# Image-Processing-Systems-Laboratory/DeepInPainting

Measured on AMD Instinct MI355X. Metric: train images/sec at 256x256, batch 8/GPU, 1/2/4/8 MI355X; IPSR layer ms, higher is better.
Workload: dtype f32; 1 GPU; BASELINE config 2: 256x256 synthetic images, 128x128 centre mask (M=256 of N=1024 feature positions), batch 8/GPU, fp32, full IPSR training step; global_batch=8, parallelism=dp1, dropout=True, conv_math=fp32, vgg16=seeded random init (no pretrained weights offline)

## Files before the change

deepinpainting_amd/csrc/smallmap.hip:

```cpp
#include <algorithm>

#include "ipsr_common.h"

namespace ipsr {

typedef float f32x16 __attribute__((ext_vector_type(16)));
typedef float f32x4v __attribute__((ext_vector_type(4)));

__global__ void __launch_bounds__(256) sm_to_cn_kernel(const float* __restrict__ x, int B, int C, int HW, int Tp, float* __restrict__ out)
{
    const int n = blockIdx.x * 256 + threadIdx.x, c = blockIdx.y;
    if (n >= Tp) return;
    float v = 0.0f;
    if (n < B * HW) { const int b = n / HW, p = n - b * HW; v = x[((size_t)b * C + c) * HW + p]; }
    out[(size_t)c * Tp + n] = v;
}

__global__ void __launch_bounds__(256) sm_to_nc_kernel(const float* __restrict__ x, int B, int C, int HW, float* __restrict__ out)
{
    const int c = blockIdx.x * 256 + threadIdx.x, n = blockIdx.y;
    if (c >= C) return;
    float v = 0.0f;
    if (n < B * HW) { const int b = n / HW, p = n - b * HW; v = x[((size_t)b * C + c) * HW + p]; }
    out[(size_t)n * C + c] = v;
// ... 354 lines not shown
    };
    auto mma = [&](const Set& s) {
#pragma unroll
        for (int u = 0; u < G; ++u)
#pragma unroll
            for (int j = 0; j < 4; ++j) acc[j] = __builtin_amdgcn_mfma_f32_32x32x2f32(s.av[u], s.b[u][j], acc[j], 0, 0, 0);
    };
    sm_stream<Set>(cdiv_dev(Pp, 2 * G), load, mma);
#pragma unroll
    for (int e = 0; e < 16; ++e) {
        const int row = (e & 3) + 8 * (e >> 2) + 4 * h;
        *reinterpret_cast<f32x4v*>(dW + (size_t)(r0 + row) * Q + q0 + 4 * m) = f32x4v{acc[0][e], acc[1][e], acc[2][e], acc[3][e]};
    }
}

constexpr int SM_WRW_GATHER_MAX_POS = 32;
static bool sm_staged(int op, int P)
{
    const int forced = debug_option(3);
    return forced == 1 || (forced != 2 && op == 1 && P > SM_WRW_GATHER_MAX_POS);
}

struct SmPlan { int P, Tp, Pp, Q, nb, ngroups, nslab, per_slab; size_t a_floats, b_floats, m_floats, total_bytes; };

static int sm_plan(int op, int B, int R, int Cq, int Ho, int Wo, int Hf, int Wf, int k, int st, int pad, int dil, SmPlan* p)
{
    if (op < 0 || op > 2) return fail(IPSR_ERR_INVALID, "small-map convolution: op %d", op);
    if (k < 1 || k > 4 || st < 1 || st > 2 || dil < 1 || pad < 0) return fail(IPSR_ERR_UNSUPPORTED, "small-map convolution: k%d s%d p%d d%d", k, st, pad, dil);
    if (Ho != (Hf + 2 * pad - dil * (k - 1) - 1) / st + 1 || Wo != (Wf + 2 * pad - dil * (k - 1) - 1) / st + 1)
        return fail(IPSR_ERR_INVALID, "small-map convolution: %dx%d is not the output grid of %dx%d under k%d s%d p%d d%d", Ho, Wo, Hf, Wf, k, st, pad, dil);
    p->P = B * Ho * Wo;
    p->Q = Cq * k * k;
    if (p->Q % 128 != 0) return fail(IPSR_ERR_UNSUPPORTED, "small-map convolution: %d x %d taps is not a multiple of 128", Cq, k * k);
    if (R % 32 != 0) return fail(IPSR_ERR_UNSUPPORTED, "small-map convolution: %d weight rows are not a multiple of 32", R);
    if (p->P > 1024) return fail(IPSR_ERR_UNSUPPORTED, "small-map convolution: %d positions (made for <= 1024)", p->P);
    const int blocks = (p->P + 31) / 32;
    p->nb = blocks >= 4 ? 4 : (blocks == 3 ? 4 : blocks);
    if (op == 0 && p->nb == 4) p->nb = 2;
    p->ngroups = (blocks + p->nb - 1) / p->nb;
    p->Tp = p->ngroups * p->nb * 32;
    p->Pp = (p->P + 1) & ~1;
    p->a_floats = p->b_floats = p->m_floats = 0;
    p->nslab = 1; p->per_slab = 0;
    const size_t w_bytes = (size_t)R * p->Q * 4;
    if (op == 0) {
        const int qb = p->Q / 128;
        const size_t slab_bytes = (size_t)p->Q * p->Tp * 4;
        const int cap = (int)std::max<size_t>(1, w_bytes / slab_bytes);
        int ns = std::max(1, std::min({R / 64, cap, (256 + qb * p->ngroups - 1) / (qb * p->ngroups)}));
        p->per_slab = (((R + 4 * ns - 1) / (4 * ns)) + 1) & ~1;
        p->nslab = (R + 4 * p->per_slab - 1) / (4 * p->per_slab);
        p->b_floats = (size_t)R * p->Tp;
        p->m_floats = (size_t)p->nslab * p->Q * p->Tp;
    } else if (op == 2) {
        const int rb = R / 32;
        const size_t slab_bytes = (size_t)R * p->Tp * 4;
        const int cap = (int)std::max<size_t>(1, w_bytes / slab_bytes);
        int ns = std::max(1, std::min({p->Q / 256, cap, (256 + rb * p->ngroups - 1) / (rb * p->ngroups)}));
// ... 16 lines not shown
    return p.total_bytes;
}

int launch_smallmap(int op, const float* a, const float* b2, float* out, int B, int R, int Cq, int Ho, int Wo, int Hf, int Wf,
                    int k, int st_, int pad, int dil, void* ws, size_t ws_bytes, hipStream_t st)
{
    SmPlan p;
    if (int rc = sm_plan(op, B, R, Cq, Ho, Wo, Hf, Wf, k, st_, pad, dil, &p)) return rc;
    if (ws_bytes < p.total_bytes) return fail(IPSR_ERR_WORKSPACE, "small-map convolution: workspace %zu < %zu", ws_bytes, p.total_bytes);
    Carver cv(ws, ws_bytes);
    float* A = cv.take<float>(p.a_floats);
    float* Bv = cv.take<float>(p.b_floats);
    float* Mo = cv.take<float>(p.m_floats);
    const size_t largest = 4 * std::max({(size_t)R * p.Q, (size_t)B * Cq * Hf * Wf, (size_t)R * p.Tp, (size_t)p.Q * p.Tp, (size_t)p.Pp * p.Q});
    if (largest >= SM_OFF) return fail(IPSR_ERR_UNSUPPORTED, "small-map convolution: an operand of %zu bytes (made for < 2 GiB)", largest);
    const bool staged = sm_staged(op, p.P);
    const SmGeo g = {p.P, R, Cq, Ho, Wo, Hf, Wf, k, st_, pad, dil};
    if (op == 0) {
        if (staged) sm_to_cn_kernel<<<dim3(cdiv(p.Tp, 256), R), 256, 0, st>>>(a, B, R, Ho * Wo, p.Tp, Bv);
        const float* in = staged ? Bv : a;
        const int HW = staged ? 0 : Ho * Wo;
        const dim3 grid(p.Q / 128, p.nslab, p.ngroups);
        if (p.nb == 1) sm_data_kernel<1><<<grid, 256, 0, st>>>(b2, in, R, p.Q, p.Tp, p.per_slab, p.P, HW, Mo);
        else sm_data_kernel<2><<<grid, 256, 0, st>>>(b2, in, R, p.Q, p.Tp, p.per_slab, p.P, HW, Mo);
        if (int rc = check_launch("sm_data_kernel")) return rc;
        const size_t total = (size_t)B * Cq * Hf * Wf;
        const unsigned cgrid = (unsigned)((total + 255) / 256);
        const size_t slab_bytes = (size_t)p.Q * p.Tp * 4, m_bytes = slab_bytes * p.nslab;
        const bool wide = !debug_option(4) && m_bytes < SM_OFF && (k == 3 || k == 4) && p.nslab <= 8;
        if (wide && k == 3) sm_col2im_wide_kernel<3, 8><<<cgrid, 256, 0, st>>>(Mo, p.nslab, (unsigned)slab_bytes, (unsigned)m_bytes, B, Cq, Hf, Wf, Ho, Wo, st_, pad, dil, p.Tp, out);
        else if (wide && p.nslab <= 4) sm_col2im_wide_kernel<4, 4><<<cgrid, 256, 0, st>>>(Mo, p.nslab, (unsigned)slab_bytes, (unsigned)m_bytes, B, Cq, Hf, Wf, Ho, Wo, st_, pad, dil, p.Tp, out);
        else if (wide) sm_col2im_wide_kernel<4, 8><<<cgrid, 256, 0, st>>>(Mo, p.nslab, (unsigned)slab_bytes, (unsigned)m_bytes, B, Cq, Hf, Wf, Ho, Wo, st_, pad, dil, p.Tp, out);
        else sm_col2im_kernel<<<cgrid, 256, 0, st>>>(Mo, p.nslab, (size_t)p.Q * p.Tp, B, Cq, Hf, Wf, Ho, Wo, k, st_, pad, dil, p.Tp, out);
        return check_launch("sm_col2im_kernel");
    }
    const int K = staged ? 0 : k;
    if (op == 2) {
        if (staged) sm_im2col_cn_kernel<<<dim3(cdiv(p.Tp, 256), p.Q), 256, 0, st>>>(a, B, Cq, Hf, Wf, Ho, Wo, k, st_, pad, dil, p.Tp, Bv);
        const float* x = staged ? Bv : a;
        const dim3 grid(R / 32, p.nslab, p.ngroups);
#define SM_FWD_K(NB)                                                                                                                                   \
    switch (K) {                                                                                                                                       \
    case 0: sm_fwd_kernel<NB, 0><<<grid, 256, 0, st>>>(b2, x, R, p.Q, p.Tp, p.per_slab, g, Mo); break;                                                 \
    case 1: sm_fwd_kernel<NB, 1><<<grid, 256, 0, st>>>(b2, x, R, p.Q, p.Tp, p.per_slab, g, Mo); break;                                                 \
    case 2: sm_fwd_kernel<NB, 2><<<grid, 256, 0, st>>>(b2, x, R, p.Q, p.Tp, p.per_slab, g, Mo); break;                                                 \
    case 3: sm_fwd_kernel<NB, 3><<<grid, 256, 0, st>>>(b2, x, R, p.Q, p.Tp, p.per_slab, g, Mo); break;                                                 \
    default: sm_fwd_kernel<NB, 4><<<grid, 256, 0, st>>>(b2, x, R, p.Q, p.Tp, p.per_slab, g, Mo); break;                                                \
    }
        if (p.nb == 1) { SM_FWD_K(1) }
        else if (p.nb == 2) { SM_FWD_K(2) }
        else { SM_FWD_K(4) }
// ... 47 lines not shown
```

deepinpainting_amd/models/IPSR.py:

```python
import os
from collections import OrderedDict

import torch

from . import networks
from .base_model import BaseModel
from .vgg16 import Vgg16
from .. import dist as ipsr_dist


class IPSR(BaseModel):
    def name(self):
        return 'IPSRModel'

    def initialize(self, opt):
        BaseModel.initialize(self, opt)
        self.opt = opt
        self.isTrain = opt.isTrain
        self.strict_reference = bool(getattr(opt, 'strict_reference', False))
        self.batch_vgg = bool(getattr(opt, 'batch_vgg', False))
        self.batch_disc = bool(getattr(opt, 'batch_disc', True))
        self.amp_bf16 = bool(getattr(opt, 'amp_bf16', False))
        from . import hipconv
        hipconv.set_conv_math(fp32=getattr(opt, 'conv_math', 'fp32'), bf16=getattr(opt, 'conv_math_bf16', 'bf16x3'))
# ... 27 lines not shown
        self.use_gpu = len(opt.gpu_ids) > 0

        self.netG, self.Cosis_list, self.Cosis_list2, self.CSA_model = networks.define_G(
            opt.input_nc_g, opt.output_nc, opt.ngf, opt.which_model_netG, opt, self.mask_global, opt.norm,
            opt.use_dropout, opt.init_type, self.gpu_ids, opt.init_gain)
        self.netP, _, _, _ = networks.define_G(
            opt.input_nc, opt.output_nc, opt.ngf, opt.which_model_netP, opt, self.mask_global, opt.norm,
            opt.use_dropout, opt.init_type, self.gpu_ids, opt.init_gain)
        self.CSA_model[0].corr_bf16 = self.amp_bf16 and bool(getattr(opt, 'bf16_corr', True)) and self.device.type == 'cuda'
        if self.isTrain:
            use_sigmoid = opt.gan_type == 'vanilla'
            self.netD = networks.define_D(opt.input_nc, opt.ndf, opt.which_model_netD, opt.n_layers_D, opt.norm,
                                          use_sigmoid, opt.init_type, self.gpu_ids, opt.init_gain)
            self.netF = networks.define_D(opt.input_nc, opt.ndf, opt.which_model_netF, opt.n_layers_D, opt.norm,
                                          use_sigmoid, opt.init_type, self.gpu_ids, opt.init_gain)

        if not self.isTrain or opt.continue_train:
            print('Loading pre-trained network!')
            self.load_network(self.netG, 'G', opt.which_epoch)
            self.load_network(self.netP, 'P', opt.which_epoch)
            if self.isTrain:
                self.load_network(self.netD, 'D', opt.which_epoch)
                self.load_network(self.netF, 'F', opt.which_epoch)

        self.criterionGAN = networks.GANLoss(gan_type=opt.gan_type)
        self.criterionL1 = torch.nn.L1Loss()
        self._gt_latent = None
        self._reducer_D = self._reducer_G = None

        if self.isTrain:
# ... 236 lines not shown
```

deepinpainting_amd/models/hipconv.py:

```python
import os
from collections import namedtuple

import torch
import torch.nn as nn
import torch.nn.functional as F

from .. import _lib, ops
from .. import dist as ipsr_dist

_FORCE = None
_MATH = {"fp32": "fp32", "bf16": "bf16x3"}


def set_conv_math(fp32=None, bf16=None):
    from .. import ops as _ops
    for key, val in (("fp32", fp32), ("bf16", bf16)):
        if val is not None:
            if val not in _ops.MATH_CODE or (key == "bf16" and val in _ops.DIRECT_PASSES):
                raise ValueError("conv math must be one of %s" % sorted(k for k in _ops.MATH_CODE if k))
            _MATH[key] = val
    _SEL.clear()


_DIRECT_DILATED = False
# ... 44 lines not shown
    v = _ENV.get(name)
    if v is None:
        v = _ENV[name] = os.environ.get(name, default)
    return v


def reload_env():
    _ENV.clear()
    _SEL.clear()


def _mode():
    return _FORCE or _env("IPSR_CONV_ENGINE", "auto")


def select(op, B, Cin, H, W, Cout, k, stride, pad, dil, bf16=False):
    key = (0, _FORCE, op, B, Cin, H, W, Cout, k, stride, pad, dil, bf16)
    eng = _SEL.get(key)
    if eng is None:
        eng = _SEL[key] = _select_any(op, (op in (ops.CONVT_FWD, ops.CONVT_BWD_DATA), B, Cin, H, W, Cout, k, stride, pad, dil), bf16)
    return eng


def _select_any(op, lay, bf16):
    eng = _select(op, lay)
    transposed, B, Cin, H, W, Cout, k, stride, pad, dil = lay
    if not bf16:
        eng = _direct_opt_in("data", eng, op, lay)
    elif not (_bf16_wins(eng, Cin, H, W, Cout) or _ENGINES[eng].fp32_copies):
        if _mode() == "auto" and _thin_wins(op, lay, True):
            eng = "thin"
        elif _mode() == "auto" and _env("IPSR_NO_THIN", "0") != "1" and op == ops.CONV_FWD and Cin == 3 and (k, stride, pad, dil) == (4, 2, 1, 1) and H * W >= 4096 \
                and engine_takes("thin_f2m", "data", op, lay, True):
            eng = "thin_f2m"
        else:
            eng = _bf16_direct(op, lay)
# ... 128 lines not shown
    return g[3] >= 1 and g[4] >= 1 and g[0] * g[3] * g[4] <= int(_env("IPSR_SMALLMAP_MAX_POS", "32")) and engine_takes("smallmap", "data", op, lay, False)


def _smallmap_wrw_wins(lay):
    transposed, B, Cin, H, W, Cout, k, stride, pad, dil = lay
    if k != 4 or stride != 2 or _env("IPSR_NO_SMALLMAP", "0") == "1":
        return False
    g = _smallmap_geometry(lay)
    return g[3] >= 1 and g[4] >= 1 and g[0] * g[3] * g[4] <= 256 and min(Cin, Cout) >= 256 and engine_takes("smallmap", "wrw", None, lay, False)


def _is_k4s1(k, stride, pad, dil):
    return k == 4 and stride == 1 and pad == 1 and dil == 1


def select_wrw(transposed, B, Cin, H, W, Cout, k, stride, pad, dil, bf16=False):
    key = (1, _FORCE, transposed, B, Cin, H, W, Cout, k, stride, pad, dil, bf16)
    eng = _SEL.get(key)
    if eng is None:
        eng = _SEL[key] = _select_wrw_any((transposed, B, Cin, H, W, Cout, k, stride, pad, dil), bf16)
    return eng


def _select_wrw_any(lay, bf16):
    transposed, B, Cin, H, W, Cout, k, stride, pad, dil = lay
    eng = _select_wrw(lay)
    thin = _mode() == "auto" and _env("IPSR_NO_THIN", "0") != "1" and pad == 1 and dil == 1 and (k, stride) in ((3, 1), (4, 2)) and H * W >= 4096 \
        and engine_takes("thin_mfma", "wrw", None, lay, bf16)
    if not bf16:
        eng = "thin_mfma" if thin and eng == "miopen" else _direct_opt_in("wrw", eng, None, lay)
    elif not (_bf16_wins(eng, Cin, H, W, Cout, True) or _ENGINES[eng].fp32_copies):
        eng = "thin_mfma" if thin else _bf16_direct_wrw(lay)
    return eng if engine_takes(eng, "wrw", None, lay, bf16) else "miopen"


def _bf16_direct_wrw(lay):
# ... 201 lines not shown
        _wino_dil_takes, bf16_io=True, sink=True, wrw_x_as_dy=True),
    "wino_s2": _Engine(
        lambda op, inp, w, lay, math, out_dtype, param: ops.conv4x4s2_winograd(_s2_mode(op), inp, w, lay[1], *_s2_geometry(lay), math=math, out_dtype=out_dtype),
        lambda x, dy, lay, math, sink: ops.conv4x4s2_winograd(ops.S2_WEIGHT_GRAD, *_fine_coarse(x, dy, lay), out=sink, math=math),
        _wino_s2_takes, bf16_io=True, sink=True, wrw_x_as_dy=True),
    "thin": _Engine(
        lambda op, inp, w, lay, math, out_dtype, param: ops.conv3x3_thin(op, inp, w, lay[1:5], lay[5], out_dtype=out_dtype),
        takes=lambda kind, op, lay, bf16: kind == "data" and lay[6:] == _K3 and ops.thin_supported(op, *lay[2:6])),
    "thin_f2m": _Engine(
        lambda op, inp, w, lay, math, out_dtype, param: ops.conv_thin_f2m_mfma(op, inp, w, lay[1:5], lay[5], lay[6], lay[7], out_dtype=out_dtype),
        takes=lambda kind, op, lay, bf16: kind == "data" and lay[8:] == (1, 1) and ops.thin_f2m_mfma_supported(op, *lay[1:8])),
    "thin_mfma": _Engine(
        None, _thin_mfma_wrw, sink=True,
        takes=lambda kind, op, lay, bf16: kind == "wrw" and lay[8:] == (1, 1) and ops.thin_wrw_mfma_supported(*lay[:8])),
    "smallmap": _Engine(
        lambda op, inp, w, lay, math, out_dtype, param: ops.conv_smallmap(_smallmap_op(op), inp, w, *_smallmap_geometry(lay)),
        lambda x, dy, lay, math, sink: ops.conv_smallmap(ops.SM_WRW, *((x, dy) if lay[0] else (dy, x)), *_smallmap_geometry(lay), out=sink),
        lambda kind, op, lay, bf16: ops.smallmap_supported(_smallmap_op(op) if kind == "data" else ops.SM_WRW, *_smallmap_geometry(lay)),
        fp32_copies=True, sink=True),
    "direct": _Engine(
        lambda op, inp, w, lay, math, out_dtype, param: ops.conv2d(op, inp, w, lay[1:5], *lay[5:]),
        takes=lambda kind, op, lay, bf16: kind == "data" and ops.conv2d_supported(op, *lay[1:])),
    "one": _Engine(
        lambda op, inp, w, lay, math, out_dtype, param: ops.conv_to_one(inp, w, lay[8]),
        lambda x, dy, lay, math, sink: ops.conv_to_one_wrw(x, dy, lay[6], lay[8], out=sink),
        lambda kind, op, lay, bf16: not lay[0] and lay[5] == 1 and (kind == "wrw" or op == ops.CONV_FWD) and ops.conv_to_one_supported(*lay[1:5], *lay[6:]),
        fp32_copies=True, sink=True),
    "bf16d": _Engine(_bf16d_data, _bf16d_wrw, _bf16d_takes, bf16_io=True, sink=True, wrw_x_as_dy=True),
    "bf16x3d": _Engine(_bf16x3d_data, takes=_bf16x3d_takes),
    "bf16x3w": _Engine(None, _bf16x3w_wrw, _bf16x3w_takes, sink=True),
    "miopen": _Engine(),
}


def _run_data(eng, op, inp, w, lay, math, out_dtype, param=None):
    e = _ENGINES[eng]
    if e.fp32_copies:
        return e.data(op, inp.float(), w, lay, math, torch.float32, param).to(out_dtype)
    return e.data(op, inp, w, lay, math, out_dtype, param)


def _run_wrw(eng, x, dy, w, lay, math):
    e = _ENGINES[eng]
    sink = ipsr_dist.grad_sink_for(w.data_ptr(), w.shape) if e.sink else None
    if e.fp32_copies:
        x, dy = x.float(), dy.float()
    elif e.wrw_x_as_dy and x.dtype != dy.dtype:
        x = x.to(dy.dtype)
    return e.wrw(x, dy, lay, math, sink)


def _miopen_forward(x, w, transposed, stride, pad, dil):
    if x.dtype != w.dtype and not torch.is_autocast_enabled():
        w = w.to(x.dtype)
    return F.conv_transpose2d(x, w, None, stride, pad, 0, 1, dil) if transposed else F.conv2d(x, w, None, stride, pad, dil)


def _miopen_backward(dy, x, w, transposed, stride, pad, dil, which):
    dt = dy.dtype
    out = torch.ops.aten.convolution_backward(dy, x if x.dtype == dt else x.to(dt), w if w.dtype == dt else w.to(dt), None, [stride, stride],
                                              [pad, pad], [dil, dil], transposed, [0, 0], 1, which)
    return out[0], (out[1].to(w.dtype) if out[1] is not None else None)


class _HipConv(torch.autograd.Function):

    @staticmethod
    def forward(ctx, x, w, lay, eng_fwd, math, act):
        transposed, B, Cin, H, W, Cout, k, stride, pad, dil = lay
        xc = x.contiguous()
        if eng_fwd == "miopen":
            y = _miopen_forward(xc, w, transposed, stride, pad, dil)
        else:
            y = _run_data(eng_fwd, ops.CONVT_FWD if transposed else ops.CONV_FWD, xc, w, lay, math, act)
        ctx.save_for_backward(xc, w)
        ctx.lay, ctx.geom = lay, (transposed, k, stride, pad, dil, Cout)
        ctx.math, ctx.bf16 = math, act == torch.bfloat16
        if _check_hook is not None:
            _check_hook("forward", eng_fwd, ctx.geom, (xc, w), y)
        return y

    @staticmethod
    def backward(ctx, dy):
        x, w = ctx.saved_tensors
        lay, math, bf16 = ctx.lay, ctx.math, ctx.bf16
        transposed, B, Cin, H, W, Cout, k, stride, pad, dil = lay
        dy = dy.contiguous()
        if bf16 and dy.dtype != torch.bfloat16:
            dy = dy.to(torch.bfloat16)
        dx = dw = None
        if ctx.needs_input_grad[0]:
            op = ops.CONVT_BWD_DATA if transposed else ops.CONV_BWD_DATA
            eng = select(op, B, Cin, H, W, Cout, k, stride, pad, dil, bf16)
            if eng == "miopen":
                dx = _miopen_backward(dy, x, w, transposed, stride, pad, dil, [True, False, False])[0]
                if dx.dtype != x.dtype:
                    dx = dx.to(x.dtype)
            else:
                dx = _run_data(eng, op, dy, w, lay, math, x.dtype)
            if _check_hook is not None:
                _check_hook("input_grad", eng, ctx.geom, (dy, x, w), dx)
        if ctx.needs_input_grad[1]:
            weng = select_wrw(transposed, B, Cin, H, W, Cout, k, stride, pad, dil, bf16)
            if weng == "miopen":
                dw = _miopen_backward(dy, x, w, transposed, stride, pad, dil, [False, True, False])[1]
            else:
                dw = _run_wrw(weng, x, dy, w, lay, math)
            if _check_hook is not None:
                _check_hook("weight_grad", weng, ctx.geom, (dy, x, w), dw)
        return dx, dw, None, None, None, None


def _geometry(m):
    ks, st, pd, dl = m.kernel_size, m.stride, m.padding, m.dilation
    if m.groups != 1 or ks[0] != ks[1] or st[0] != st[1] or pd[0] != pd[1] or dl[0] != dl[1] or isinstance(pd, str):
        return None
    if isinstance(m, nn.ConvTranspose2d) and tuple(m.output_padding) != (0, 0):
        return None
    if getattr(m, "padding_mode", "zeros") != "zeros":
        return None
    return ks[0], st[0], pd[0], dl[0]


def _layer_of(m, x, w):
    g = _geometry(m)
    if g is None or not x.is_cuda or x.dim() != 4 or w.dtype != torch.float32 or x.dtype not in (torch.float32, torch.bfloat16):
        return None
    amp = _amp_bf16()
    if not amp and torch.is_autocast_enabled():
        return None
    transposed = isinstance(m, nn.ConvTranspose2d)
    B, Cin, H, W = x.shape
    return (transposed, B, Cin, H, W, w.shape[1] if transposed else w.shape[0]) + g, amp or x.dtype == torch.bfloat16


def conv_math(bf16):
    return _MATH["bf16" if bf16 else "fp32"]


def _engines_of(lay, bf16, dx=True, dw=True):
    transposed, B, Cin, H, W, Cout, k, stride, pad, dil = lay
    fop, bop = (ops.CONVT_FWD, ops.CONVT_BWD_DATA) if transposed else (ops.CONV_FWD, ops.CONV_BWD_DATA)
    return (select(fop, B, Cin, H, W, Cout, k, stride, pad, dil, bf16),
            select(bop, B, Cin, H, W, Cout, k, stride, pad, dil, bf16) if dx else "miopen",
            select_wrw(transposed, B, Cin, H, W, Cout, k, stride, pad, dil, bf16) if dw else "miopen")


def any_engine(m, x):
    lb = _layer_of(m, x, m.weight)
    if lb is None:
        return False
    return _engines_of(*lb) != ("miopen",) * 3


def conv_nobias(m, x, weight=None):
    w = m.weight if weight is None else weight
    lb = _layer_of(m, x, w)
    if lb is not None:
        lay, bf16 = lb
        act = torch.bfloat16 if bf16 else torch.float32
        math = _MATH["bf16" if bf16 else "fp32"]
        grad = torch.is_grad_enabled()
        engs = _engines_of(lay, bf16, grad and x.requires_grad, grad and w.requires_grad)
        if grad and (x.requires_grad or w.requires_grad):
            if engs != ("miopen",) * 3:
                return _HipConv.apply(x, w, lay, engs[0], math, act)
        elif engs[0] != "miopen":
            return _run_data(engs[0], ops.CONVT_FWD if lay[0] else ops.CONV_FWD, x.contiguous(), w.detach(), lay, math, act, param=w)
    if isinstance(m, nn.ConvTranspose2d):
        return F.conv_transpose2d(x, w, None, m.stride, m.padding, m.output_padding, m.groups, m.dilation)
    return F.conv2d(x, w, None, m.stride, m.padding, m.dilation, m.groups)
```

deepinpainting_amd/ops.py:

```python
import contextlib
import threading
import weakref
from collections import namedtuple

import torch

from . import _lib

_ws_cache = {}


def _stream():
    return torch._C._cuda_getCurrentRawStream(torch._C._cuda_getDevice())


def _workspace(nbytes, device):
    key = (device.index, _stream())
    buf = _ws_cache.get(key)
    if buf is None or buf.numel() < nbytes:
        buf = torch.empty(max(int(nbytes), 1 << 20), dtype=torch.uint8, device=device)
        _ws_cache[key] = buf
    return buf


# ... 858 lines not shown
    Cs = small.shape[1]
    if tuple(small.shape) != (B, Cs, Hb * stride, Wb * stride):
        raise RuntimeError("conv_thin_wrw_mfma: narrow tensor %s does not match wide %s at stride %d" % (tuple(small.shape), tuple(big.shape), stride))
    L = _lib.lib()
    g = _result(out, (Kb, Cs, k, k), torch.float32, x.device, "conv_thin_wrw_mfma")
    ws = _probed_workspace(L, L.ipsr_conv_thin_wrw_mfma_workspace_bytes(B, Kb, Cs, Hb, Wb, k, stride), x.device,
                           "ipsr_conv_thin_wrw_mfma: Kb=%d Cs=%d %dx%d k%d s%d", (Kb, Cs, Hb, Wb, k, stride))
    _lib.check(L.ipsr_conv_thin_wrw_mfma(big.data_ptr(), small.data_ptr(), g.data_ptr(), B, Kb, Cs, Hb, Wb, k, stride, int(big.dtype == torch.bfloat16) | (2 if small.dtype == torch.bfloat16 else 0),
                                         ws.data_ptr(), ws.numel(), _stream()), "ipsr_conv_thin_wrw_mfma")
    return g


SM_DATA, SM_WRW, SM_FWD = 0, 1, 2


def smallmap_supported(op, B, R, Cq, Ho, Wo, Hf, Wf, k, stride, pad, dil):
    return _lib.lib().ipsr_conv_smallmap_workspace_bytes(op, B, R, Cq, Ho, Wo, Hf, Wf, k, stride, pad, dil) > 0


def conv_smallmap(op, a, b, B, R, Cq, Ho, Wo, Hf, Wf, k, stride, pad, dil, out=None):
    a = _req(a, torch.float32, "operand a")
    b = _req(b, torch.float32, "operand b")
    coarse, fine, wsh = (B, R, Ho, Wo), (B, Cq, Hf, Wf), (R, Cq, k, k)
    want = {SM_DATA: (coarse, wsh, fine), SM_WRW: (coarse, fine, wsh), SM_FWD: (fine, wsh, coarse)}[op]
    if tuple(a.shape) != want[0] or tuple(b.shape) != want[1]:
        raise RuntimeError("conv_smallmap op %d: operands %s / %s do not match %s / %s" % (op, tuple(a.shape), tuple(b.shape), want[0], want[1]))
    out = _result(out, want[2], torch.float32, a.device, "conv_smallmap")
    L = _lib.lib()
    ws = _probed_workspace(L, L.ipsr_conv_smallmap_workspace_bytes(op, B, R, Cq, Ho, Wo, Hf, Wf, k, stride, pad, dil), a.device,
                           "ipsr_conv_smallmap: op %d R=%d Cq=%d %dx%d -> %dx%d k%d s%d p%d d%d", (op, R, Cq, Hf, Wf, Ho, Wo, k, stride, pad, dil))
    _lib.check(L.ipsr_conv_smallmap(op, a.data_ptr(), b.data_ptr(), out.data_ptr(), B, R, Cq, Ho, Wo, Hf, Wf, k, stride, pad, dil,
                                    ws.data_ptr(), ws.numel(), _stream()), "ipsr_conv_smallmap")
    return out


def conv3x3_winograd_wrw(transposed, x, dy, Cout, out=None, math=None):
    x, x_bf = _act(x, "conv input")
    dy, dy_bf = _act(dy, "grad_output")
    if x_bf != dy_bf:
        raise TypeError("conv3x3_winograd_wrw: x and dy must have the same dtype")
    B, Cin, H, W = x.shape
    if tuple(dy.shape) != (B, Cout, H, W):
        raise RuntimeError("conv3x3_winograd_wrw: grad_output %s does not match %s" % (tuple(dy.shape), (B, Cout, H, W)))
# ... 104 lines not shown
```

deepinpainting_amd/options.py:

```python


class Option(object):
    def __init__(self, **overrides):
        self.batchSize = 1
        self.fineSize = 256
        self.input_nc = 3
        self.input_nc_g = 6
        self.output_nc = 3
        self.ngf = 64
        self.ndf = 64
        self.which_model_netD = 'basic'
        self.which_model_netF = 'feature'
        self.which_model_netG = 'unet_ipsr'
        self.which_model_netP = 'unet_256'
        self.triple_weight = 1
        self.name = 'IPSR_inpainting'
        self.n_layers_D = '3'
        self.gpu_ids = [0]
        self.model = 'ipsr_net'
        self.checkpoints_dir = './checkpoints'
        self.norm = 'instance'
        self.fixed_mask = 1
        self.use_dropout = True
        self.init_type = 'normal'
# ... 17 lines not shown
        self.display_freq = 1000
        self.print_freq = 50
        self.save_latest_freq = 5000
        self.save_epoch_freq = 1
        self.continue_train = False
        self.epoch_count = 1
        self.phase = 'train'
        self.which_epoch = ''
        self.niter = 20
        self.niter_decay = 100
        self.beta1 = 0.5
        self.lr = 0.0002
        self.lr_policy = 'lambda'
        self.lr_decay_iters = 50
        self.isTrain = True
        for k, v in overrides.items():
            setattr(self, k, v)
```

include/ipsr_hip.h:

```cpp
#ifndef IPSR_HIP_H
#define IPSR_HIP_H

#include <stddef.h>
#include <stdint.h>

#ifdef __cplusplus
extern "C" {
#endif

#define IPSR_OK                 0
#define IPSR_ERR_INVALID       -1
#define IPSR_ERR_UNSUPPORTED   -2
#define IPSR_ERR_WORKSPACE     -3
#define IPSR_ERR_LAUNCH        -4

int ipsr_abi_version(void);
const char* ipsr_last_error(void);

size_t ipsr_feat_mask_workspace_bytes(int H, int W, int layers);
int ipsr_feat_mask(const uint8_t* mask, int H, int W, int layers, float threshold,
                   uint8_t* feat, void* ws, size_t ws_bytes, void* stream);

int ipsr_index_prep(const uint8_t* feat, int h, int w, int patch, int stride, int mask_thred,
                    int32_t* flag , int32_t* mask_point_idx , int32_t* count ,
// ... 81 lines not shown
int ipsr_conv3x3_winograd_wrw(int transposed, const float* x, const float* dy, float* dw, int B, int Cin, int H, int W, int Cout,
                              void* ws, size_t ws_bytes, void* stream);

size_t ipsr_conv4x4_dilated_winograd_workspace_bytes(int mode, int B, int Cin, int H, int W, int Cout);
int ipsr_conv4x4_dilated_winograd(int mode, const float* a, const float* b, float* out, int B, int Cin, int H, int W, int Cout,
                                  void* ws, size_t ws_bytes, void* stream);

size_t ipsr_conv4x4_winograd_workspace_bytes(int geom, int mode, int B, int Cin, int H, int W, int Cout);
int ipsr_conv4x4_winograd(int geom, int mode, const float* a, const float* b, float* out, int B, int Cin, int H, int W, int Cout,
                          void* ws, size_t ws_bytes, void* stream);

size_t ipsr_conv4x4s2_winograd_workspace_bytes(int mode, int B, int Kc, int Cf, int nh, int nw);
int ipsr_conv4x4s2_winograd(int mode, const float* a, const float* b, float* out, int B, int Kc, int Cf, int nh, int nw,
                            void* ws, size_t ws_bytes, void* stream);

size_t ipsr_conv_smallmap_workspace_bytes(int op, int B, int R, int Cq, int Ho, int Wo, int Hf, int Wf, int k, int stride, int pad, int dil);
int ipsr_conv_smallmap(int op, const float* a, const float* b, float* out, int B, int R, int Cq, int Ho, int Wo, int Hf, int Wf,
                       int k, int stride, int pad, int dil, void* ws, size_t ws_bytes, void* stream);

int ipsr_conv3x3_thin(int op, const float* in, const float* w, const float* bias, int relu, float* out, int B, int I, int O, int H, int W,
                      long so, long si, int flip, void* stream);
size_t ipsr_conv3x3_thin_wrw_workspace_bytes(int B, int Cb, int Cs, int H, int W);
int ipsr_conv3x3_thin_io(int op, const void* in, const float* w, const float* bias, int relu, void* out, int B, int I, int O, int H, int W,
                         long so, long si, int flip, int io, void* stream);
int ipsr_conv3x3_thin_wrw_io(const void* big, const void* small, float* g, int B, int Cb, int Cs, int H, int W, int io,
                             void* ws, size_t ws_bytes, void* stream);
int ipsr_conv_thin_f2m_mfma_supported(int B, int Cs, int O, int Ho, int Wo, int k, int stride);
int ipsr_conv_thin_f2m_mfma(const void* in, const float* w, const float* bias, int relu, void* out, int B, int Cs, int O, int Ho, int Wo, int k, int stride,
                            long so, long si, int flip, int io, void* stream);
size_t ipsr_conv_thin_wrw_mfma_workspace_bytes(int B, int Kb, int Cs, int Hb, int Wb, int k, int stride);
// ... 78 lines not shown
```

Before: 353.7 images/sec.

## Add tiled MFMA small-map conv kernel and route MIOpen k4 layers to it

Adds a 128x128x16 LDS-tiled MFMA GEMM kernel for small-map convolution forward and backward-data. It double-buffers the weight tiles, uses direct global-to-LDS DMA in the backward-data path, and split-K partials, with a sum or col2im pass afterwards. The Python selector gains a per-module 'reach' option, on by default up to 1024 positions. With it, k=4 layers with at least 256 channels that previously fell back to MIOpen are sent to the smallmap engine (tiled or streaming) according to a position-count regime table. The aim is to beat MIOpen on mid-sized maps, at the cost of extra split-K partial traffic and a reduction pass.

```diff
diff --git a/deepinpainting_amd/csrc/smallmap.hip b/deepinpainting_amd/csrc/smallmap.hip
--- a/deepinpainting_amd/csrc/smallmap.hip
+++ b/deepinpainting_amd/csrc/smallmap.hip
@@ -392,6 +392,142 @@
     }
 }
 
+typedef const __attribute__((address_space(1))) void* sm_gptr_t;
+typedef __attribute__((address_space(3))) void* sm_lptr_t;
+constexpr int SMT_BM = 128, SMT_BN = 128, SMT_BK = 16, SMT_NBUF = 2, SMT_SLOT = 2 * SMT_BK * SMT_BM;
+
+template <bool FWD, int K>
+__global__ void __launch_bounds__(256, 4) sm_tiled_kernel(const float* __restrict__ Wm, const float* __restrict__ X, int R, int Q, int Tp, int m_tiles,
+                                                          int ksplit, int stages_per_split, int nstage, SmGeo g, float* __restrict__ part)
+{
+    __shared__ __attribute__((aligned(16))) float lds[SMT_NBUF * SMT_SLOT];
+    const int tid = threadIdx.x;
+    const int lane = tid & 63, wave = __builtin_amdgcn_readfirstlane(tid >> 6);
+    const int wm = wave >> 1, wn = wave & 1, r = lane & 31, h = lane >> 5;
+    const int M = FWD ? R : Q;
+
+    const unsigned L = xcd_remap(blockIdx.x, gridDim.x);
+    const int mt = L % m_tiles, ks = (L / m_tiles) % ksplit, nt = L / (m_tiles * ksplit);
+    const int m0 = mt * SMT_BM, n0 = nt * SMT_BN;
+    const int s_lo = ks * stages_per_split;
+    const int ns = min(nstage, s_lo + stages_per_split) - s_lo;
+
+    const int gpar = wave >> 1, gn = n0 + (tid & 127);
+    const int HW = g.Ho * g.Wo;
+    const __amdgpu_buffer_rsrc_t xrs = sm_rsrc(X, (unsigned)(g.P / HW) * (FWD ? g.C * g.Hf * g.Wf : R * HW) * 4u);
+    const SmPos pos(g, gn);
+    const unsigned icol = gn < g.P ? (unsigned)((gn / HW) * R * HW + gn % HW) * 4u : SM_OFF;
+    float breg[8];
+    auto gather = [&](int s) {
+        const unsigned row0 = (unsigned)((s_lo + s) * SMT_BK + 8 * gpar);
+#pragma unroll
+        for (int jj = 0; jj < 8; ++jj)
+            breg[jj] = sm_ld(xrs, FWD ? sm_tap_off<K>(g, pos, row0 + jj, 1u) : icol + (row0 + jj) * (unsigned)HW * 4u);
+    };
+    auto store_b = [&](int s) {
+        float* bt = lds + (s & (SMT_NBUF - 1)) * SMT_SLOT + SMT_BK * SMT_BM + (tid & 127);
+#pragma unroll
+        for (int jj = 0; jj < 8; ++jj) bt[(jj + 8 * gpar) * SMT_BM] = breg[jj];
+    };
+
+    const int dma_row = lane >> 5, dma_col = (lane & 31) * 4;
+    const float* wbase = Wm + (size_t)s_lo * SMT_BK * Q + m0 + dma_col;
+    auto dma_piece = [&](int s, int q) {
+        const int slot = (s & (SMT_NBUF - 1)) * SMT_SLOT + q * 2 * SMT_BM;
+        const float* src = wbase + ((size_t)s * SMT_BK + 2 * q + dma_row) * Q;
+        __builtin_amdgcn_global_load_lds((sm_gptr_t)src, (sm_lptr_t)&lds[slot], 16, 0, 0);
+    };
+    auto dma_stage = [&](int s) {
+        dma_piece(s, wave);
+        dma_piece(s, wave + 4);
+    };
+    const __amdgpu_buffer_rsrc_t wrs = sm_rsrc(Wm, (unsigned)R * Q * 4u);
+    const int arow = tid >> 2, akc = tid & 3;
+    unsigned aoff[2];
+#pragma unroll
+    for (int i = 0; i < 2; ++i) {
+        const int row = m0 + arow + 64 * i;
+        aoff[i] = sm_off((unsigned)(min(row, R - 1) * Q + s_lo * SMT_BK + 4 * akc) * 4u, row < R);
+    }
+    f32x4v areg[2];
+    auto load_a = [&](int s) {
+#pragma unroll
+        for (int i = 0; i < 2; ++i) areg[i] = sm_ld4(wrs, aoff[i] + (unsigned)(s * SMT_BK) * 4u);
+    };
+    auto store_a = [&](int s) {
+        float* at = lds + (s & (SMT_NBUF - 1)) * SMT_SLOT + 4 * akc * SMT_BM + arow;
+#pragma unroll
+        for (int i = 0; i < 2; ++i)
+#pragma unroll
+            for (int j = 0; j < 4; ++j) at[j * SMT_BM + 64 * i] = areg[i][j];
+    };
+
+    f32x16 acc[2][2];
+#pragma unroll
+    for (int i = 0; i < 2; ++i)
+#pragma unroll
+        for (int j = 0; j < 2; ++j)
+#pragma unroll
+            for (int e = 0; e < 16; ++e) acc[i][j][e] = 0.0f;
+
+    if constexpr (FWD) load_a(0);
+    else dma_stage(0);
+    gather(0);
+    if constexpr (FWD) store_a(0);
+    store_b(0);
+    asm volatile("s_waitcnt vmcnt(0)" ::: "memory");
+    asm volatile("s_waitcnt lgkmcnt(0)" ::: "memory");
+    __builtin_amdgcn_s_barrier();
+
+    for (int s = 0; s < ns; ++s) {
+        const int cur = s & (SMT_NBUF - 1);
+        const bool more = s + 1 < ns;
+        if (more) {
+            if constexpr (FWD) load_a(s + 1);
+            gather(s + 1);
+        }
+        const float* ta = lds + cur * SMT_SLOT + h * SMT_BM + wm * 32 + r;
+        const float* tb = lds + cur * SMT_SLOT + SMT_BK * SMT_BM + h * SMT_BM + wn * 32 + r;
+        float fa0[3], fa1[3], fb0[3], fb1[3];
+        fa0[0] = ta[0]; fa1[0] = ta[64]; fb0[0] = tb[0]; fb1[0] = tb[64];
+#pragma unroll
+        for (int kk = 0; kk < SMT_BK / 2; ++kk) {
+            const int cs = kk % 3, nx = (kk + 1) % 3;
+            if (kk + 1 < SMT_BK / 2) {
+                const int ro = (kk + 1) * 2 * SMT_BM;
+                fa0[nx] = ta[ro]; fa1[nx] = ta[ro + 64]; fb0[nx] = tb[ro]; fb1[nx] = tb[ro + 64];
+            }
+            if (!FWD && more && kk < 2) dma_piece(s + 1, wave + 4 * kk);
+            __builtin_amdgcn_sched_barrier(0);
+            acc[0][0] = __builtin_amdgcn_mfma_f32_32x32x2f32(fa0[cs], fb0[cs], acc[0][0], 0, 0, 0);
+            acc[0][1] = __builtin_amdgcn_mfma_f32_32x32x2f32(fa0[cs], fb1[cs], acc[0][1], 0, 0, 0);
+            acc[1][0] = __builtin_amdgcn_mfma_f32_32x32x2f32(fa1[cs], fb0[cs], acc[1][0], 0, 0, 0);
+            acc[1][1] = __builtin_amdgcn_mfma_f32_32x32x2f32(fa1[cs], fb1[cs], acc[1][1], 0, 0, 0);
+            __builtin_amdgcn_sched_barrier(0);
+        }
+        asm volatile("s_waitcnt vmcnt(0)" ::: "memory");
+        if (more) {
+            if constexpr (FWD) store_a(s + 1);
+            store_b(s + 1);
+        }
+        asm volatile("s_waitcnt lgkmcnt(0)" ::: "memory");
+        __builtin_amdgcn_s_barrier();
+    }
+
+    float* dst = part + (size_t)ks * M * Tp;
+#pragma unroll
+    for (int jn = 0; jn < 2; ++jn) {
+        const int n = n0 + wn * 32 + jn * 64 + r;
+#pragma unroll
+        for (int im = 0; im < 2; ++im) {
+            const int mb = m0 + wm * 32 + im * 64;
+            if (mb >= M) continue;
+#pragma unroll
+            for (int e = 0; e < 16; ++e) dst[(size_t)(mb + (e & 3) + 8 * (e >> 2) + 4 * h) * Tp + n] = acc[im][jn][e];
+        }
+    }
+}
+
 constexpr int SM_WRW_GATHER_MAX_POS = 32;
 static bool sm_staged(int op, int P)
 {
@@ -399,11 +535,19 @@
     return forced == 1 || (forced != 2 && op == 1 && P > SM_WRW_GATHER_MAX_POS);
 }
 
-struct SmPlan { int P, Tp, Pp, Q, nb, ngroups, nslab, per_slab; size_t a_floats, b_floats, m_floats, total_bytes; };
+constexpr int SM_TILED = 16, SM_TILED_MIN_POS = 33;
+static bool sm_tiled(int op, int flags, int k, int P)
+{
+    return (flags & SM_TILED) && !debug_option(5) && (op == 0 || op == 2) && (k == 3 || k == 4) && P >= SM_TILED_MIN_POS;
+}
+
+struct SmPlan { int P, Tp, Pp, Q, nb, ngroups, nslab, per_slab, m_tiles, nstage; bool tiled; size_t a_floats, b_floats, m_floats, total_bytes; };
 
 static int sm_plan(int op, int B, int R, int Cq, int Ho, int Wo, int Hf, int Wf, int k, int st, int pad, int dil, SmPlan* p)
 {
-    if (op < 0 || op > 2) return fail(IPSR_ERR_INVALID, "small-map convolution: op %d", op);
+    const int flags = op & ~3;
+    op &= 3;
+    if ((flags & ~SM_TILED) || op > 2) return fail(IPSR_ERR_INVALID, "small-map convolution: op %d", op | flags);
     if (k < 1 || k > 4 || st < 1 || st > 2 || dil < 1 || pad < 0) return fail(IPSR_ERR_UNSUPPORTED, "small-map convolution: k%d s%d p%d d%d", k, st, pad, dil);
     if (Ho != (Hf + 2 * pad - dil * (k - 1) - 1) / st + 1 || Wo != (Wf + 2 * pad - dil * (k - 1) - 1) / st + 1)
         return fail(IPSR_ERR_INVALID, "small-map convolution: %dx%d is not the output grid of %dx%d under k%d s%d p%d d%d", Ho, Wo, Hf, Wf, k, st, pad, dil);
@@ -420,6 +564,23 @@
     p->Pp = (p->P + 1) & ~1;
     p->a_floats = p->b_floats = p->m_floats = 0;
     p->nslab = 1; p->per_slab = 0;
+    p->m_tiles = p->nstage = 0;
+    p->tiled = sm_tiled(op, flags, k, p->P);
+    if (p->tiled) {
+        const int M = op == 0 ? p->Q : R, red = op == 0 ? R : p->Q;
+        p->ngroups = (p->P + SMT_BN - 1) / SMT_BN;
+        p->Tp = p->ngroups * SMT_BN;
+        p->m_tiles = (M + SMT_BM - 1) / SMT_BM;
+        p->nstage = red / SMT_BK;
+        const int tiles = p->m_tiles * p->ngroups;
+        int ks = std::max(1, std::min({op == 0 ? 4 : 32, p->nstage / 8, (512 + tiles - 1) / tiles}));
+        if (debug_option(6) > 0) ks = std::min(debug_option(6), p->nstage);
+        p->per_slab = (p->nstage + ks - 1) / ks;
+        p->nslab = (p->nstage + p->per_slab - 1) / p->per_slab;
+        p->m_floats = (size_t)p->nslab * M * p->Tp;
+        p->total_bytes = align_up(p->m_floats * 4, 256) + 768;
+        return IPSR_OK;
+    }
     const size_t w_bytes = (size_t)R * p->Q * 4;
     if (op == 0) {
         const int qb = p->Q / 128;
@@ -466,16 +627,23 @@
     float* Mo = cv.take<float>(p.m_floats);
     const size_t largest = 4 * std::max({(size_t)R * p.Q, (size_t)B * Cq * Hf * Wf, (size_t)R * p.Tp, (size_t)p.Q * p.Tp, (size_t)p.Pp * p.Q});
     if (largest >= SM_OFF) return fail(IPSR_ERR_UNSUPPORTED, "small-map convolution: an operand of %zu bytes (made for < 2 GiB)", largest);
+    op &= 3;
     const bool staged = sm_staged(op, p.P);
     const SmGeo g = {p.P, R, Cq, Ho, Wo, Hf, Wf, k, st_, pad, dil};
+    const unsigned tgrid = (unsigned)(p.m_tiles * p.nslab * p.ngroups);
     if (op == 0) {
-        if (staged) sm_to_cn_kernel<<<dim3(cdiv(p.Tp, 256), R), 256, 0, st>>>(a, B, R, Ho * Wo, p.Tp, Bv);
-        const float* in = staged ? Bv : a;
-        const int HW = staged ? 0 : Ho * Wo;
-        const dim3 grid(p.Q / 128, p.nslab, p.ngroups);
-        if (p.nb == 1) sm_data_kernel<1><<<grid, 256, 0, st>>>(b2, in, R, p.Q, p.Tp, p.per_slab, p.P, HW, Mo);
-        else sm_data_kernel<2><<<grid, 256, 0, st>>>(b2, in, R, p.Q, p.Tp, p.per_slab, p.P, HW, Mo);
-        if (int rc = check_launch("sm_data_kernel")) return rc;
+        if (p.tiled) {
+            sm_tiled_kernel<false, 4><<<tgrid, 256, 0, st>>>(b2, a, R, p.Q, p.Tp, p.m_tiles, p.nslab, p.per_slab, p.nstage, g, Mo);
+            if (int rc = check_launch("sm_tiled_kernel")) return rc;
+        } else {
+            if (staged) sm_to_cn_kernel<<<dim3(cdiv(p.Tp, 256), R), 256, 0, st>>>(a, B, R, Ho * Wo, p.Tp, Bv);
+            const float* in = staged ? Bv : a;
+            const int HW = staged ? 0 : Ho * Wo;
+            const dim3 grid(p.Q / 128, p.nslab, p.ngroups);
+            if (p.nb == 1) sm_data_kernel<1><<<grid, 256, 0, st>>>(b2, in, R, p.Q, p.Tp, p.per_slab, p.P, HW, Mo);
+            else sm_data_kernel<2><<<grid, 256, 0, st>>>(b2, in, R, p.Q, p.Tp, p.per_slab, p.P, HW, Mo);
+            if (int rc = check_launch("sm_data_kernel")) return rc;
+        }
         const size_t total = (size_t)B * Cq * Hf * Wf;
         const unsigned cgrid = (unsigned)((total + 255) / 256);
         const size_t slab_bytes = (size_t)p.Q * p.Tp * 4, m_bytes = slab_bytes * p.nslab;
@@ -487,6 +655,14 @@
         return check_launch("sm_col2im_kernel");
     }
     const int K = staged ? 0 : k;
+    if (op == 2 && p.tiled) {
+        if (k == 3) sm_tiled_kernel<true, 3><<<tgrid, 256, 0, st>>>(b2, a, R, p.Q, p.Tp, p.m_tiles, p.nslab, p.per_slab, p.nstage, g, Mo);
+        else sm_tiled_kernel<true, 4><<<tgrid, 256, 0, st>>>(b2, a, R, p.Q, p.Tp, p.m_tiles, p.nslab, p.per_slab, p.nstage, g, Mo);
+        if (int rc = check_launch("sm_tiled_kernel")) return rc;
+        const size_t total = (size_t)B * R * Ho * Wo;
+        sm_sum_to_nchw_kernel<<<(unsigned)((total + 255) / 256), 256, 0, st>>>(Mo, p.nslab, (size_t)R * p.Tp, B, R, Ho * Wo, p.Tp, out);
+        return check_launch("sm_sum_to_nchw_kernel");
+    }
     if (op == 2) {
         if (staged) sm_im2col_cn_kernel<<<dim3(cdiv(p.Tp, 256), p.Q), 256, 0, st>>>(a, B, Cq, Hf, Wf, Ho, Wo, k, st_, pad, dil, p.Tp, Bv);
         const float* x = staged ? Bv : a;
diff --git a/deepinpainting_amd/models/IPSR.py b/deepinpainting_amd/models/IPSR.py
--- a/deepinpainting_amd/models/IPSR.py
+++ b/deepinpainting_amd/models/IPSR.py
@@ -65,6 +65,12 @@
                                           use_sigmoid, opt.init_type, self.gpu_ids, opt.init_gain)
             self.netF = networks.define_D(opt.input_nc, opt.ndf, opt.which_model_netF, opt.n_layers_D, opt.norm,
                                           use_sigmoid, opt.init_type, self.gpu_ids, opt.init_gain)
+
+        reach = 0 if self.amp_bf16 else int(getattr(opt, 'smallmap_reach', 1024))
+        for net in (self.netG, self.netP) + ((self.netD, self.netF) if self.isTrain else ()):
+            for mod in net.modules():
+                if isinstance(mod, (torch.nn.Conv2d, torch.nn.ConvTranspose2d)):
+                    mod.smallmap_reach = reach or None
 
         if not self.isTrain or opt.continue_train:
             print('Loading pre-trained network!')
diff --git a/deepinpainting_amd/models/hipconv.py b/deepinpainting_amd/models/hipconv.py
--- a/deepinpainting_amd/models/hipconv.py
+++ b/deepinpainting_amd/models/hipconv.py
@@ -82,12 +82,60 @@
     return _FORCE or _env("IPSR_CONV_ENGINE", "auto")
 
 
-def select(op, B, Cin, H, W, Cout, k, stride, pad, dil, bf16=False):
+def select(op, B, Cin, H, W, Cout, k, stride, pad, dil, bf16=False, reach=None):
     key = (0, _FORCE, op, B, Cin, H, W, Cout, k, stride, pad, dil, bf16)
     eng = _SEL.get(key)
     if eng is None:
         eng = _SEL[key] = _select_any(op, (op in (ops.CONVT_FWD, ops.CONVT_BWD_DATA), B, Cin, H, W, Cout, k, stride, pad, dil), bf16)
-    return eng
+    return _reached("data", key, eng, op, bf16, reach) if reach else eng
+
+
+
+
+def _reach_regime(kind, op, lay):
+    transposed, B, Cin, H, W, Cout, k, stride, pad, dil = lay
+    g = _smallmap_geometry(lay)
+    pos = g[0] * g[3] * g[4] if g[3] >= 1 and g[4] >= 1 else 0
+    if pos < 1:
+        return None
+    if kind == "wrw":
+        return None
+    if pos <= 32:
+        return None
+    if k != 4:
+        return None
+    if pos <= 128:
+        return "stream"
+    fwd = _smallmap_op(op) == ops.SM_FWD
+    if pos <= 256:
+        return "tiled" if fwd else "stream"
+    if pos <= 512:
+        return None if fwd and g[1] > 512 else "tiled"
+    return "tiled" if fwd else None
+
+
+def _reached(kind, key, eng, op, bf16, reach):
+    if eng != "miopen" or bf16:
+        return eng
+    rkey = key + (int(reach),)
+    hit = _SEL.get(rkey)
+    if hit is None:
+        lay = ((op in (ops.CONVT_FWD, ops.CONVT_BWD_DATA),) if kind == "data" else ()) + key[3 if kind == "data" else 2:-1]
+        transposed, B, Cin, H, W, Cout, k, stride, pad, dil = lay
+        g = _smallmap_geometry(lay)
+        regime = _reach_regime(kind, op, lay)
+        ok = _mode() == "auto" and _env("IPSR_NO_SMALLMAP", "0") != "1" and regime is not None and k in (3, 4) and min(Cin, Cout) >= 256 \
+            and g[0] * g[3] * g[4] <= int(reach) and bool(_ENGINES["smallmap"].takes(kind, op, lay, False, tiled=regime == "tiled"))
+        hit = _SEL[rkey] = "smallmap" if ok else eng
+    return hit
+
+
+def _via_reach(kind, op, lay, bf16, reach):
+    if not reach or _reach_regime(kind, op, lay) != "tiled":
+        return False
+    if kind == "data":
+        return select(op, *lay[1:], bf16) != "smallmap" and select(op, *lay[1:], bf16, reach=reach) == "smallmap"
+    return select_wrw(*lay, bf16) != "smallmap" and select_wrw(*lay, bf16, reach=reach) == "smallmap"
 
 
 def _select_any(op, lay, bf16):
@@ -246,12 +294,12 @@
     return k == 4 and stride == 1 and pad == 1 and dil == 1
 
 
-def select_wrw(transposed, B, Cin, H, W, Cout, k, stride, pad, dil, bf16=False):
+def select_wrw(transposed, B, Cin, H, W, Cout, k, stride, pad, dil, bf16=False, reach=None):
     key = (1, _FORCE, transposed, B, Cin, H, W, Cout, k, stride, pad, dil, bf16)
     eng = _SEL.get(key)
     if eng is None:
         eng = _SEL[key] = _select_wrw_any((transposed, B, Cin, H, W, Cout, k, stride, pad, dil), bf16)
-    return eng
+    return _reached("wrw", key, eng, None, bf16, reach) if reach else eng
 
 
 def _select_wrw_any(lay, bf16):
@@ -483,9 +531,11 @@
         None, _thin_mfma_wrw, sink=True,
         takes=lambda kind, op, lay, bf16: kind == "wrw" and lay[8:] == (1, 1) and ops.thin_wrw_mfma_supported(*lay[:8])),
     "smallmap": _Engine(
-        lambda op, inp, w, lay, math, out_dtype, param: ops.conv_smallmap(_smallmap_op(op), inp, w, *_smallmap_geometry(lay)),
-        lambda x, dy, lay, math, sink: ops.conv_smallmap(ops.SM_WRW, *((x, dy) if lay[0] else (dy, x)), *_smallmap_geometry(lay), out=sink),
-        lambda kind, op, lay, bf16: ops.smallmap_supported(_smallmap_op(op) if kind == "data" else ops.SM_WRW, *_smallmap_geometry(lay)),
+        lambda op, inp, w, lay, math, out_dtype, param, tiled=False: ops.conv_smallmap(_smallmap_op(op), inp, w, *_smallmap_geometry(lay), tiled=tiled),
+        lambda x, dy, lay, math, sink, tiled=False: ops.conv_smallmap(ops.SM_WRW, *((x, dy) if lay[0] else (dy, x)), *_smallmap_geometry(lay), out=sink,
+                                                                       tiled=tiled),
+        lambda kind, op, lay, bf16, tiled=False: ops.smallmap_supported(_smallmap_op(op) if kind == "data" else ops.SM_WRW, *_smallmap_geometry(lay),
+                                                                         tiled=tiled),
         fp32_copies=True, sink=True),
     "direct": _Engine(
         lambda op, inp, w, lay, math, out_dtype, param: ops.conv2d(op, inp, w, lay[1:5], *lay[5:]),
@@ -502,21 +552,22 @@
 }
 
 
-def _run_data(eng, op, inp, w, lay, math, out_dtype, param=None):
+def _run_data(eng, op, inp, w, lay, math, out_dtype, param=None, tiled=False):
     e = _ENGINES[eng]
+    kw = {"tiled": True} if tiled else {}
     if e.fp32_copies:
-        return e.data(op, inp.float(), w, lay, math, torch.float32, param).to(out_dtype)
-    return e.data(op, inp, w, lay, math, out_dtype, param)
-
-
-def _run_wrw(eng, x, dy, w, lay, math):
+        return e.data(op, inp.float(), w, lay, math, torch.float32, param, **kw).to(out_dtype)
+    return e.data(op, inp, w, lay, math, out_dtype, param, **kw)
+
+
+def _run_wrw(eng, x, dy, w, lay, math, tiled=False):
     e = _ENGINES[eng]
     sink = ipsr_dist.grad_sink_for(w.data_ptr(), w.shape) if e.sink else None
     if e.fp32_copies:
         x, dy = x.float(), dy.float()
     elif e.wrw_x_as_dy and x.dtype != dy.dtype:
         x = x.to(dy.dtype)
-    return e.wrw(x, dy, lay, math, sink)
+    return e.wrw(x, dy, lay, math, sink, **({"tiled": True} if tiled else {}))
 
 
 def _miopen_forward(x, w, transposed, stride, pad, dil):
@@ -535,16 +586,17 @@
 class _HipConv(torch.autograd.Function):
 
     @staticmethod
-    def forward(ctx, x, w, lay, eng_fwd, math, act):
+    def forward(ctx, x, w, lay, eng_fwd, math, act, reach=None):
         transposed, B, Cin, H, W, Cout, k, stride, pad, dil = lay
         xc = x.contiguous()
         if eng_fwd == "miopen":
             y = _miopen_forward(xc, w, transposed, stride, pad, dil)
         else:
-            y = _run_data(eng_fwd, ops.CONVT_FWD if transposed else ops.CONV_FWD, xc, w, lay, math, act)
+            fop = ops.CONVT_FWD if transposed else ops.CONV_FWD
+            y = _run_data(eng_fwd, fop, xc, w, lay, math, act, tiled=eng_fwd == "smallmap" and _via_reach("data", fop, lay, act == torch.bfloat16, reach))
         ctx.save_for_backward(xc, w)
         ctx.lay, ctx.geom = lay, (transposed, k, stride, pad, dil, Cout)
-        ctx.math, ctx.bf16 = math, act == torch.bfloat16
+        ctx.math, ctx.bf16, ctx.reach = math, act == torch.bfloat16, reach
         if _check_hook is not None:
             _check_hook("forward", eng_fwd, ctx.geom, (xc, w), y)
         return y
@@ -552,7 +604,7 @@
     @staticmethod
     def backward(ctx, dy):
         x, w = ctx.saved_tensors
-        lay, math, bf16 = ctx.lay, ctx.math, ctx.bf16
+        lay, math, bf16, reach = ctx.lay, ctx.math, ctx.bf16, ctx.reach
         transposed, B, Cin, H, W, Cout, k, stride, pad, dil = lay
         dy = dy.contiguous()
         if bf16 and dy.dtype != torch.bfloat16:
@@ -560,24 +612,24 @@
         dx = dw = None
         if ctx.needs_input_grad[0]:
             op = ops.CONVT_BWD_DATA if transposed else ops.CONV_BWD_DATA
-            eng = select(op, B, Cin, H, W, Cout, k, stride, pad, dil, bf16)
+            eng = select(op, B, Cin, H, W, Cout, k, stride, pad, dil, bf16, reach=reach)
             if eng == "miopen":
                 dx = _miopen_backward(dy, x, w, transposed, stride, pad, dil, [True, False, False])[0]
                 if dx.dtype != x.dtype:
                     dx = dx.to(x.dtype)
             else:
-                dx = _run_data(eng, op, dy, w, lay, math, x.dtype)
+                dx = _run_data(eng, op, dy, w, lay, math, x.dtype, tiled=eng == "smallmap" and _via_reach("data", op, lay, bf16, reach))
             if _check_hook is not None:
                 _check_hook("input_grad", eng, ctx.geom, (dy, x, w), dx)
         if ctx.needs_input_grad[1]:
-            weng = select_wrw(transposed, B, Cin, H, W, Cout, k, stride, pad, dil, bf16)
+            weng = select_wrw(transposed, B, Cin, H, W, Cout, k, stride, pad, dil, bf16, reach=reach)
             if weng == "miopen":
                 dw = _miopen_backward(dy, x, w, transposed, stride, pad, dil, [False, True, False])[1]
             else:
-                dw = _run_wrw(weng, x, dy, w, lay, math)
+                dw = _run_wrw(weng, x, dy, w, lay, math, tiled=weng == "smallmap" and _via_reach("wrw", None, lay, bf16, reach))
             if _check_hook is not None:
                 _check_hook("weight_grad", weng, ctx.geom, (dy, x, w), dw)
-        return dx, dw, None, None, None, None
+        return dx, dw, None, None, None, None, None
 
 
 def _geometry(m):
@@ -607,19 +659,19 @@
     return _MATH["bf16" if bf16 else "fp32"]
 
 
-def _engines_of(lay, bf16, dx=True, dw=True):
+def _engines_of(lay, bf16, dx=True, dw=True, reach=None):
     transposed, B, Cin, H, W, Cout, k, stride, pad, dil = lay
     fop, bop = (ops.CONVT_FWD, ops.CONVT_BWD_DATA) if transposed else (ops.CONV_FWD, ops.CONV_BWD_DATA)
-    return (select(fop, B, Cin, H, W, Cout, k, stride, pad, dil, bf16),
-            select(bop, B, Cin, H, W, Cout, k, stride, pad, dil, bf16) if dx else "miopen",
-            select_wrw(transposed, B, Cin, H, W, Cout, k, stride, pad, dil, bf16) if dw else "miopen")
+    return (select(fop, B, Cin, H, W, Cout, k, stride, pad, dil, bf16, reach=reach),
+            select(bop, B, Cin, H, W, Cout, k, stride, pad, dil, bf16, reach=reach) if dx else "miopen",
+            select_wrw(transposed, B, Cin, H, W, Cout, k, stride, pad, dil, bf16, reach=reach) if dw else "miopen")
 
 
 def any_engine(m, x):
     lb = _layer_of(m, x, m.weight)
     if lb is None:
         return False
-    return _engines_of(*lb) != ("miopen",) * 3
+    return _engines_of(*lb, reach=getattr(m, "smallmap_reach", None)) != ("miopen",) * 3
 
 
 def conv_nobias(m, x, weight=None):
@@ -630,12 +682,15 @@
         act = torch.bfloat16 if bf16 else torch.float32
         math = _MATH["bf16" if bf16 else "fp32"]
         grad = torch.is_grad_enabled()
-        engs = _engines_of(lay, bf16, grad and x.requires_grad, grad and w.requires_grad)
+        reach = getattr(m, "smallmap_reach", None)
+        engs = _engines_of(lay, bf16, grad and x.requires_grad, grad and w.requires_grad, reach)
         if grad and (x.requires_grad or w.requires_grad):
             if engs != ("miopen",) * 3:
-                return _HipConv.apply(x, w, lay, engs[0], math, act)
+                return _HipConv.apply(x, w, lay, engs[0], math, act, reach)
         elif engs[0] != "miopen":
-            return _run_data(engs[0], ops.CONVT_FWD if lay[0] else ops.CONV_FWD, x.contiguous(), w.detach(), lay, math, act, param=w)
+            fop = ops.CONVT_FWD if lay[0] else ops.CONV_FWD
+            return _run_data(engs[0], fop, x.contiguous(), w.detach(), lay, math, act, param=w,
+                             tiled=engs[0] == "smallmap" and _via_reach("data", fop, lay, bf16, reach))
     if isinstance(m, nn.ConvTranspose2d):
         return F.conv_transpose2d(x, w, None, m.stride, m.padding, m.output_padding, m.groups, m.dilation)
     return F.conv2d(x, w, None, m.stride, m.padding, m.dilation, m.groups)
diff --git a/deepinpainting_amd/ops.py b/deepinpainting_amd/ops.py
--- a/deepinpainting_amd/ops.py
+++ b/deepinpainting_amd/ops.py
@@ -896,11 +896,14 @@
 SM_DATA, SM_WRW, SM_FWD = 0, 1, 2
 
 
-def smallmap_supported(op, B, R, Cq, Ho, Wo, Hf, Wf, k, stride, pad, dil):
-    return _lib.lib().ipsr_conv_smallmap_workspace_bytes(op, B, R, Cq, Ho, Wo, Hf, Wf, k, stride, pad, dil) > 0
-
-
-def conv_smallmap(op, a, b, B, R, Cq, Ho, Wo, Hf, Wf, k, stride, pad, dil, out=None):
+SM_TILED = 16
+
+
+def smallmap_supported(op, B, R, Cq, Ho, Wo, Hf, Wf, k, stride, pad, dil, tiled=False):
+    return _lib.lib().ipsr_conv_smallmap_workspace_bytes(op | (SM_TILED if tiled else 0), B, R, Cq, Ho, Wo, Hf, Wf, k, stride, pad, dil) > 0
+
+
+def conv_smallmap(op, a, b, B, R, Cq, Ho, Wo, Hf, Wf, k, stride, pad, dil, out=None, tiled=False):
     a = _req(a, torch.float32, "operand a")
     b = _req(b, torch.float32, "operand b")
     coarse, fine, wsh = (B, R, Ho, Wo), (B, Cq, Hf, Wf), (R, Cq, k, k)
@@ -909,6 +912,7 @@
         raise RuntimeError("conv_smallmap op %d: operands %s / %s do not match %s / %s" % (op, tuple(a.shape), tuple(b.shape), want[0], want[1]))
     out = _result(out, want[2], torch.float32, a.device, "conv_smallmap")
     L = _lib.lib()
+    op |= SM_TILED if tiled else 0
     ws = _probed_workspace(L, L.ipsr_conv_smallmap_workspace_bytes(op, B, R, Cq, Ho, Wo, Hf, Wf, k, stride, pad, dil), a.device,
                            "ipsr_conv_smallmap: op %d R=%d Cq=%d %dx%d -> %dx%d k%d s%d p%d d%d", (op, R, Cq, Hf, Wf, Ho, Wo, k, stride, pad, dil))
     _lib.check(L.ipsr_conv_smallmap(op, a.data_ptr(), b.data_ptr(), out.data_ptr(), B, R, Cq, Ho, Wo, Hf, Wf, k, stride, pad, dil,
diff --git a/deepinpainting_amd/options.py b/deepinpainting_amd/options.py
--- a/deepinpainting_amd/options.py
+++ b/deepinpainting_amd/options.py
@@ -55,5 +55,6 @@
         self.lr_policy = 'lambda'
         self.lr_decay_iters = 50
         self.isTrain = True
+        self.smallmap_reach = 1024
         for k, v in overrides.items():
             setattr(self, k, v)
diff --git a/include/ipsr_hip.h b/include/ipsr_hip.h
--- a/include/ipsr_hip.h
+++ b/include/ipsr_hip.h
@@ -119,6 +119,7 @@
 int ipsr_conv4x4s2_winograd(int mode, const float* a, const float* b, float* out, int B, int Kc, int Cf, int nh, int nw,
                             void* ws, size_t ws_bytes, void* stream);
 
+#define IPSR_SMALLMAP_TILED 16
 size_t ipsr_conv_smallmap_workspace_bytes(int op, int B, int R, int Cq, int Ho, int Wo, int Hf, int Wf, int k, int stride, int pad, int dil);
 int ipsr_conv_smallmap(int op, const float* a, const float* b, float* out, int B, int R, int Cq, int Ho, int Wo, int Hf, int Wf,
                        int k, int stride, int pad, int dil, void* ws, size_t ws_bytes, void* stream);
```

Result: faster. 358.9 images/sec, median of 6 (+1.5%).
